# wolearyc/ramannoodle

Measured on AMD Instinct MI355X. Metric: structures/sec (GNN polarizability eval), higher is better.
Workload: dtype f32

## Files before the change

ramannoodle_amd/csrc/api.hip:

```cpp
#include <hip/hip_runtime.h>

#include <algorithm>
#include <chrono>
#include <cmath>
#include <cstdarg>
#include <cstdio>
#include <cstdlib>
#include <cstring>
#include <functional>
#include <memory>
#include <mutex>
#include <string>
#include <thread>
#include <vector>

#include "../../include/rn_potgnn.h"
#include "graph_plan.hpp"
#include "host_runtime.hpp"
#include "increments.hpp"
#include "kernels.hpp"
#include "weight_layout.hpp"

using namespace rn;

// ... 2476 lines not shown
      }
      launch_gather_segments(w, h->step_seg.as<long long>(), (int)(seg.size() / 3), h->step_stage.as<float>(), st);
      HIP_TRY(hipMemcpyAsync(h->step_host, h->step_stage.p, (size_t)total * sizeof(float), hipMemcpyDeviceToHost, st));
      HIP_TRY(hipStreamSynchronize(st));
      for (size_t i = 0; i < seg.size(); i += 3)
        std::memcpy(h->packed.data() + seg[i], h->step_host + seg[i + 1], (size_t)seg[i + 2] * sizeof(float));
    }
    HIP_TRY(hipStreamSynchronize(st));
    h->grads_on_device = false;
    h->train_S = 0;
    h->host_stale = true;
    refresh_pass_flags<float>(h);
    refresh_mfma_mode(h);
    check_ps_fail(h);
  });
}

int rn_potgnn_get_weights(rn_potgnn *h, float *weights, size_t num_weights) {
  if (!h || !weights || num_weights != h->lay.weight_count()) {
    set_error(h, "invalid arguments to get_weights");
    return RN_ERR_INVALID_ARGUMENT;
  }
  return guarded(h, [&]() {
    sync_host(h);
    unpack_weights<float>(h->lay, h->packed.data(), weights, true);
  });
}

int rn_potgnn_set_stat_reducer(rn_potgnn *h, rn_potgnn_reduce_fn fn, void *ctx) {
  if (!h) return RN_ERR_INVALID_ARGUMENT;
  std::lock_guard<std::recursive_mutex> hold(h->lock);
  h->reducer = fn;
  h->reducer_ctx = ctx;
  return RN_OK;
}

double rn_potgnn_train_row_count(const rn_potgnn *h) {
  if (!h) return 0.0;
  std::lock_guard<std::recursive_mutex> hold(h->lock);
  return h->bn_count;
}

int rn_potgnn_train_backward(rn_potgnn *h, const float *dvec6, float *grads) {
  const Checked c = check_pending(h, dvec6 && grads, "train_backward", kHostF32,
                                  "train_backward needs a preceding train_forward (an evaluation or Jacobian call in "
                                  "between discards its tape)");
  if (c.rc != kGo) return c.rc;
  return guarded(h, [&]() { train_backward<float>(h, dvec6, grads); });
}

int rn_potgnn_radius_graph(const double *lattice, const double *positions, int32_t num_atoms,
                           double cutoff, int device, uint8_t *adjacency) {
  if (!lattice || !positions || !adjacency || num_atoms <= 0 || !(cutoff > 0)) {
    set_error<rn_potgnn>(nullptr, "invalid arguments to radius_graph");
    return RN_ERR_INVALID_ARGUMENT;
  }
  int ndev = 0;
  if (hipGetDeviceCount(&ndev) != hipSuccess || device < 0 || device >= ndev) {
    set_error<rn_potgnn>(nullptr, "no usable HIP device (count=%d, requested=%d)", ndev, device);
    return RN_ERR_NO_DEVICE;
  }
  return guarded<rn_potgnn>(nullptr, [&]() {
    HIP_TRY(hipSetDevice(device));
    const size_t n = (size_t)num_atoms;
    DeviceBuf lat, pos, adj;
    lat.ensure(9 * sizeof(double));
    pos.ensure(n * 3 * sizeof(double));
    adj.ensure(n * n);
    HIP_TRY(hipMemcpy(lat.p, lattice, 9 * sizeof(double), hipMemcpyHostToDevice));
    HIP_TRY(hipMemcpy(pos.p, positions, n * 3 * sizeof(double), hipMemcpyHostToDevice));
    launch_radius_graph(lat.as<double>(), pos.as<double>(), num_atoms, (float)cutoff,
                        adj.as<unsigned char>(), nullptr);
    HIP_TRY(hipGetLastError());
    HIP_TRY(hipDeviceSynchronize());
    HIP_TRY(hipMemcpy(adjacency, adj.p, n * n, hipMemcpyDeviceToHost));
  });
}

int rn_potgnn_config_flags(const rn_potgnn *h) {
  if (!h) return -1;
  std::lock_guard<std::recursive_mutex> hold(h->lock);
  int flags = (h->plan.use_fused ? 1 : 0) | ((h->plan.use_fused && h->mfma_f16) ? 4 : 0) | (h->plan.use_narrow ? 8 : 0) |
              ((h->plan.use_fused && h->mfma_range_fallback) ? 16 : 0);
  {
    bool ps = h->plan.use_fused && h->plan.use_ps && !h->f32.pass.empty();
    for (const auto &p : h->f32.pass) ps = ps && (p.c3_fast & 1);
    flags |= ps ? 256 : 0;
  }
  {
    static const bool centred = !(getenv("RN_POTGNN_NODE_CENTRED") && atoi(getenv("RN_POTGNN_NODE_CENTRED")) == 0);
    const bool atom = h->plan.use_fused && h->plan.use_node_fused && h->mfma_f16 && centred && h->g.na_num > 0;
    flags |= atom ? 512 : 0;
    flags |= (atom && (flags & 256) && h->plan.use_readout_fused && h->want_pair_rows && !h->keep_stages) ? 1024 : 0;
    flags |= ((flags & 1024) && h->want_c2_pairs && c2_rows_fit(h)) ? 2048 : 0;
  }
  bool fast = !h->f32.pass.empty();
  for (const auto &p : h->f32.pass) fast = fast && !h->plan.use_narrow && (p.c3_fast & (h->plan.use_fused ? 1 : 2));
  return flags | (fast ? 2 : 0);
}

int rn_potgnn_debug_ps_schedule(const int32_t *rb, const int32_t *re, int32_t num_destinations, int32_t back, int32_t ring_tiles,
                                int32_t *window) {
  if (!rb || !re || num_destinations < 0 || back < 1 || back > 8 || ring_tiles < 1 || ring_tiles > 64) return RN_ERR_INVALID_ARGUMENT;
  int w = 0;
  const bool ok = edge_ps_tile_ok(rb, re, num_destinations, back, ring_tiles, &w);
  if (window) *window = w;
  return ok ? 1 : 0;
}

int64_t rn_potgnn_num_triplets(const rn_potgnn *h) { return h ? h->g.T : -1; }

int rn_potgnn_debug_triplets(rn_potgnn *h, int32_t *idx_i, int32_t *idx_j, int32_t *idx_k,
                             int32_t *slot5, int32_t *slot6) {
  if (!h || !idx_i || !idx_j || !idx_k || !slot5 || !slot6) return RN_ERR_INVALID_ARGUMENT;
  return guarded(h, [&]() {
    const size_t T = (size_t)h->g.T;
    if (T == 0) return;
    DeviceBuf buf;
    buf.ensure(5 * T * sizeof(int));
    int *p = buf.as<int>();
    launch_enum_triplets(h->g, p, p + T, p + 2 * T, p + 3 * T, p + 4 * T, nullptr);
    HIP_TRY(hipGetLastError());
    HIP_TRY(hipDeviceSynchronize());
    int32_t *outs[5] = {idx_i, idx_j, idx_k, slot5, slot6};
    for (int k = 0; k < 5; ++k)
      HIP_TRY(hipMemcpy(outs[k], p + k * T, T * sizeof(int), hipMemcpyDeviceToHost));
  });
}

int rn_potgnn_debug_stage(rn_potgnn *h, int stage, int index, float *out, size_t out_capacity,
                          int64_t *rows, int64_t *cols) {
  if (!h || !out || !rows || !cols) return RN_ERR_INVALID_ARGUMENT;
  std::lock_guard<std::recursive_mutex> hold(h->lock);
  if (h->last_was_f64) {
    set_error(h, "debug_stage only reads the float32 path");
    return RN_ERR_UNSUPPORTED;
  }
  const int S = h->last_chunk_structs;
  Precision<float> &P = h->f32;
  return guarded(h, [&]() {
    HIP_TRY(hipDeviceSynchronize());
    const float *src = nullptr;
    int64_t r = 0, c = 0, ld = 0;
    const int64_t ME = (int64_t)S * h->g.E, MN = (int64_t)S * h->g.N;
    if (stage == 0) {
      src = P.lanes[0].unit4.as<float>(); r = ME; c = 4; ld = 4;
    } else if (stage == 1 || stage == 2) {
      if ((!h->keep_stages && !h->snap_pairs) || index < 0 || index > h->cfg.num_message_passes)
        throw HipError{hipErrorInvalidValue, "stage snapshots need RN_POTGNN_KEEP_STAGES=1 or 2"};
      if (stage == 1) { src = P.snap_node[index].as<float>(); r = MN; c = h->d.Fn; ld = h->d.FnP; }
      else { src = P.snap_edge[index].as<float>(); r = ME; c = h->d.Fe; ld = h->d.FeP; }
    } else if (stage == 3) {
      src = P.lanes[0].bufA.as<float>(); r = ME; c = 12; ld = 32;
    } else {
      throw HipError{hipErrorInvalidValue, "unknown stage"};
    }
    if ((size_t)(r * c) > out_capacity) throw HipError{hipErrorInvalidValue, "out_capacity too small"};
    if (stage == 2 && h->snap_pairs && h->last_pair_rows) {
      std::vector<_Float16> raw((size_t)r * 128);
      HIP_TRY(hipMemcpy(raw.data(), src, raw.size() * sizeof(_Float16), hipMemcpyDeviceToHost));
      for (int64_t i = 0; i < r; ++i)
        for (int64_t k = 0; k < c; ++k) {
          const _Float16 *grp = raw.data() + i * 128 + (k >> 3) * 16;
          out[i * c + k] = (float)grp[k & 7] + (float)grp[8 + (k & 7)];
        }
      *rows = r;
      *cols = c;
      return;
    }
    HIP_TRY(hipMemcpy2D(out, c * sizeof(float), src, ld * sizeof(float), c * sizeof(float), r,
                        hipMemcpyDeviceToHost));
    if (h->last_in_order && r == ME && stage != 1) {
      std::vector<float> tmp(out, out + r * c);
      const int E = h->g.E;
      for (int64_t s = 0; s < S; ++s)
        for (int e = 0; e < E; ++e)
          std::memcpy(out + (s * E + e) * c, tmp.data() + (s * E + h->plan.in_pos[e]) * c, (size_t)c * sizeof(float));
    }
    *rows = r;
    *cols = c;
  });
}

int rn_potgnn_set_profiling(rn_potgnn *h, int enabled) {
  if (!h) return RN_ERR_INVALID_ARGUMENT;
  std::lock_guard<std::recursive_mutex> hold(h->lock);
  resolve_timers(h);
  h->profiling = enabled;
  for (int k = 0; k < K_COUNT; ++k) {
    h->k_ms[k] = 0;
    h->k_launches[k] = 0;
  }
  return RN_OK;
}

int rn_potgnn_kernel_times(rn_potgnn *h, const char **names, double *millis, int64_t *launches,
                           int cap) {
  if (!h || !names || !millis || !launches) return RN_ERR_INVALID_ARGUMENT;
  std::lock_guard<std::recursive_mutex> hold(h->lock);
  (void)hipSetDevice(h->cfg.device);
  resolve_timers(h);
  int n = 0;
  for (int k = 0; k < K_COUNT && n < cap; ++k, ++n) {
    names[n] = kKernelNames[k];
    millis[n] = h->k_ms[k];
    launches[n] = h->k_launches[k];
  }
  return n;
}

}
```

ramannoodle_amd/csrc/kernels_agg.hip:

```cpp
#include <algorithm>
#include <cstdlib>

#include "device_utils.hpp"
#include "kernels.hpp"

namespace rn {

#define RN_DISPATCH_LG(FP, PAD, CALL)                                   \
  do {                                                                  \
    switch ((FP) / 4) {                                                 \
      case 4:  if (PAD) { CALL(4, true); }  else { CALL(4, false); }  break;  \
      case 8:  if (PAD) { CALL(8, true); }  else { CALL(8, false); }  break;  \
      case 16: if (PAD) { CALL(16, true); } else { CALL(16, false); } break;  \
      case 32: if (PAD) { CALL(32, true); } else { CALL(32, false); } break;  \
    }                                                                   \
  } while (0)

template <typename T>
__global__ void setup_kernel(const T *emb, const T *W2, const T *b2, const T *W4,
                             const T *b4, int K, Dims d, T *node_table, const T *b0,
                             const T *bn_w, const T *bn_b, const T *bn_rm, const T *bn_rv,
                             T *scale0, T *shift0) {
  extern __shared__ unsigned char smem_raw[];
  T *h = reinterpret_cast<T *>(smem_raw);
  const int Fn = d.Fn;
  for (int i = threadIdx.x; i < K * Fn; i += blockDim.x) {
    int k = i / Fn, o = i % Fn;
    T acc = b2[o];
    for (int c = 0; c < Fn; ++c) acc += ssp(emb[k * Fn + c]) * W2[o * Fn + c];
    h[i] = ssp(acc);
  }
  __syncthreads();
  for (int i = threadIdx.x; i < K * d.FnP; i += blockDim.x) {
    int k = i / d.FnP, o = i % d.FnP;
    T acc = 0;
    if (o < Fn) {
      acc = b4[o];
      for (int c = 0; c < Fn; ++c) acc += h[k * Fn + c] * W4[o * Fn + c];
    }
    node_table[i] = acc;
  }
  for (int o = threadIdx.x; o < d.FeP; o += blockDim.x) {
    T sc = 0, sh = 0;
    if (o < d.Fe) {
      T inv = (T)1 / sqrt(bn_rv[o] + (T)1e-5);
      sc = inv * bn_w[o];
      sh = (b0[o] - bn_rm[o]) * sc + bn_b[o];
    }
    scale0[o] = sc;
    shift0[o] = sh;
  }
}

template <typename T>
void launch_setup(const T *emb, const T *W2, const T *b2, const T *W4, const T *b4, int K,
                  Dims d, T *node_table, const T *b0, const T *bn_w, const T *bn_b,
                  const T *bn_rm, const T *bn_rv, T *scale0, T *shift0, hipStream_t st) {
  size_t lds = (size_t)K * d.Fn * sizeof(T);
  setup_kernel<T><<<1, 256, lds, st>>>(emb, W2, b2, W4, b4, K, d, node_table, b0, bn_w, bn_b,
                                       bn_rm, bn_rv, scale0, shift0);
}
template void launch_setup<float>(const float *, const float *, const float *, const float *,
                                  const float *, int, Dims, float *, const float *,
                                  const float *, const float *, const float *, const float *,
                                  float *, float *, hipStream_t);
template void launch_setup<double>(const double *, const double *, const double *,
                                   const double *, const double *, int, Dims, double *,
                                   const double *, const double *, const double *,
                                   const double *, const double *, double *, double *,
                                   hipStream_t);

template <typename T, typename PT>
__global__ __launch_bounds__(256) void geom_rbf_kernel(const PT *__restrict__ pos, int S,
                                                       Graph g, const T *__restrict__ lat_base,
                                                       int lat_stride,
                                                       const T *__restrict__ offs, T coef,
                                                       Dims d, T *__restrict__ unit4,
                                                       T *__restrict__ edge0, int in_order) {
  __shared__ T sdist[256];
  const int64_t total = (int64_t)S * g.E;
  const int64_t r0 = (int64_t)blockIdx.x * 256;
  const int64_t row = r0 + threadIdx.x;
  T dist = 0;
  if (row < total) {
    const int s = (int)(row / g.E);
    const int e = in_order ? g.in_edge[(int)(row % g.E)] : (int)(row % g.E);
    const int a = g.edge_a[e], b = g.edge_b[e];
    const T *lat = lat_base + (int64_t)s * lat_stride;
    const PT *pa = pos + ((int64_t)s * g.N + a) * 3;
    const PT *pb = pos + ((int64_t)s * g.N + b) * 3;
    T f[3];
#pragma unroll
    for (int k = 0; k < 3; ++k) f[k] = wrap_min_image((T)pb[k] - (T)pa[k]);
    T c[3];
#pragma unroll
    for (int k = 0; k < 3; ++k) c[k] = f[0] * lat[k] + f[1] * lat[3 + k] + f[2] * lat[6 + k];
    dist = sqrt(c[0] * c[0] + c[1] * c[1] + c[2] * c[2]);
    T *u = unit4 + row * 4;
    u[0] = c[0] / dist;
    u[1] = c[1] / dist;
    u[2] = c[2] / dist;
    u[3] = dist;
  }
  sdist[threadIdx.x] = dist;
  __syncthreads();
  const int c4n = d.FeP / 4;
  for (int i = threadIdx.x; i < 256 * c4n; i += 256) {
    const int r = i / c4n, q = i % c4n;
    if (r0 + r >= total) break;
    const T dd = sdist[r];
    Vec4<T> o;
#pragma unroll
    for (int j = 0; j < 4; ++j) {
      const int col = 4 * q + j;
      T x = dd - offs[col];
      if constexpr (sizeof(T) == 4)
        o.v[j] = (col < d.Fe) ? __builtin_amdgcn_exp2f((coef * 1.4426950408889634f) * (x * x)) : 0.0f;
      else
        o.v[j] = (col < d.Fe) ? exp(coef * (x * x)) : (T)0;
    }
    store4(edge0 + (r0 + r) * d.FeP + 4 * q, o);
  }
}

template <typename T>
void launch_geom_rbf(const double *pos, int S, const Graph &g, const T *lattice, int lat_stride,
                     const T *offsets, T coef, Dims d, T *unit4, T *edge0, hipStream_t st, bool in_order) {
  const int64_t total = (int64_t)S * g.E;
  if (total == 0) return;
  geom_rbf_kernel<T, double><<<(unsigned)((total + 255) / 256), 256, 0, st>>>(pos, S, g, lattice, lat_stride,
                                                                              offsets, coef, d, unit4, edge0, in_order ? 1 : 0);
}
void launch_geom_rbf_pos32(const float *pos, int S, const Graph &g, const float *lattice, int lat_stride,
                           const float *offsets, float coef, Dims d, float *unit4, float *edge0, hipStream_t st, bool in_order) {
  const int64_t total = (int64_t)S * g.E;
  if (total == 0) return;
  geom_rbf_kernel<float, float><<<(unsigned)((total + 255) / 256), 256, 0, st>>>(pos, S, g, lattice, lat_stride,
                                                                                 offsets, coef, d, unit4, edge0, in_order ? 1 : 0);
}
template <typename PT>
__global__ __launch_bounds__(256) void geom_rbf_pairs_kernel(const PT *__restrict__ pos, int S, Graph g,
                                                             const float *__restrict__ lat_base, int lat_stride,
                                                             const float *__restrict__ offs, float coef, Dims d,
                                                             float *__restrict__ unit4, float *__restrict__ edge0) {
  typedef _Float16 h8 __attribute__((ext_vector_type(8)));
  __shared__ float sdist[256];
  const int64_t total = (int64_t)S * g.E;
  const int64_t r0 = (int64_t)blockIdx.x * 256;
  const int64_t row = r0 + threadIdx.x;
  float dist = 0;
  if (row < total) {
    const int s = (int)(row / g.E), e = (int)(row % g.E);
    const int a = g.edge_a[e], b = g.edge_b[e];
    const float *lat = lat_base + (int64_t)s * lat_stride;
    const PT *pa = pos + ((int64_t)s * g.N + a) * 3;
    const PT *pb = pos + ((int64_t)s * g.N + b) * 3;
    float f[3];
#pragma unroll
    for (int k = 0; k < 3; ++k) f[k] = wrap_min_image((float)pb[k] - (float)pa[k]);
    float c[3];
#pragma unroll
    for (int k = 0; k < 3; ++k) c[k] = f[0] * lat[k] + f[1] * lat[3 + k] + f[2] * lat[6 + k];
    dist = sqrt(c[0] * c[0] + c[1] * c[1] + c[2] * c[2]);
    float *u = unit4 + row * 4;
    u[0] = c[0] / dist;
    u[1] = c[1] / dist;
    u[2] = c[2] / dist;
    u[3] = dist;
  }
  sdist[threadIdx.x] = dist;
  __syncthreads();
  for (int i = threadIdx.x; i < 256 * 8; i += 256) {
    const int r = i >> 3, m = i & 7;
    if (r0 + r >= total) break;
    const float dd = sdist[r];
    h8 hi, lo;
#pragma unroll
    for (int j = 0; j < 8; ++j) {
      const int col = 8 * m + j;
      const float x = dd - offs[col];
      const float v = (col < d.Fe) ? __builtin_amdgcn_exp2f((coef * 1.4426950408889634f) * (x * x)) : 0.0f;
      hi[j] = (_Float16)v;
      lo[j] = (_Float16)(v - (float)hi[j]);
    }
    h8 *o = reinterpret_cast<h8 *>(edge0 + (r0 + r) * 64 + 8 * m);
    o[0] = hi;
    o[1] = lo;
  }
}
void launch_geom_rbf_pairs(const double *pos, int S, const Graph &g, const float *lattice, int lat_stride, const float *offsets,
                           float coef, Dims d, float *unit4, float *edge0, hipStream_t st) {
  const int64_t total = (int64_t)S * g.E;
  if (total == 0) return;
  geom_rbf_pairs_kernel<double><<<(unsigned)((total + 255) / 256), 256, 0, st>>>(pos, S, g, lattice, lat_stride, offsets, coef, d,
                                                                                 unit4, edge0);
}
void launch_geom_rbf_pairs_pos32(const float *pos, int S, const Graph &g, const float *lattice, int lat_stride, const float *offsets,
                                 float coef, Dims d, float *unit4, float *edge0, hipStream_t st) {
  const int64_t total = (int64_t)S * g.E;
  if (total == 0) return;
  geom_rbf_pairs_kernel<float><<<(unsigned)((total + 255) / 256), 256, 0, st>>>(pos, S, g, lattice, lat_stride, offsets, coef, d,
                                                                                unit4, edge0);
}
template void launch_geom_rbf<float>(const double *, int, const Graph &, const float *, int,
                                     const float *, float, Dims, float *, float *, hipStream_t, bool);
template void launch_geom_rbf<double>(const double *, int, const Graph &, const double *, int,
                                      const double *, double, Dims, double *, double *,
                                      hipStream_t, bool);

template <typename T>
__global__ void node_init_kernel(const T *__restrict__ table, int S, Graph g, Dims d,
                                 T *__restrict__ node, const int *__restrict__ types) {
  const int c4n = d.FnP / 4;
  const int64_t total = (int64_t)S * g.N * c4n;
  for (int64_t i = (int64_t)blockIdx.x * blockDim.x + threadIdx.x; i < total;
       i += (int64_t)gridDim.x * blockDim.x) {
    const int q = (int)(i % c4n);
    const int64_t rown = i / c4n;
    const int n = (int)(rown % g.N);
    const int ty = types ? types[rown] : g.atom_type[n];
    store4(node + rown * d.FnP + 4 * q, load4<T>(table + ty * d.FnP + 4 * q));
  }
}
template <typename T>
void launch_node_init(const T *table, int S, const Graph &g, Dims d, T *node, const int *types, hipStream_t st) {
  const int64_t total = (int64_t)S * g.N * (d.FnP / 4);
  if (total == 0) return;
  unsigned blocks = (unsigned)((total + 255) / 256);
  if (blocks > 4096) blocks = 4096;
  node_init_kernel<T><<<blocks, 256, 0, st>>>(table, S, g, d, node, types);
}
template void launch_node_init<float>(const float *, int, const Graph &, Dims, float *, const int *, hipStream_t);
template void launch_node_init<double>(const double *, int, const Graph &, Dims, double *, const int *,
                                       hipStream_t);

template <int LG, bool PAD, typename T>
__global__ __launch_bounds__(256) void node_agg_kernel(const T *__restrict__ npc1,
                                                       const T *__restrict__ bc1,
                                                       const T *__restrict__ node_in,
                                                       T *__restrict__ node_out, int S, Graph g,
                                                       Dims d, PassW<T> w) {
  constexpr int FP = LG * 4;
  const int64_t gid = ((int64_t)blockIdx.x * 256 + threadIdx.x) / LG;
  const int q = threadIdx.x % LG;
  if (gid >= (int64_t)S * g.N) return;
  const int s = (int)(gid / g.N), b = (int)(gid % g.N);
  const int nvalid = min(max(d.Fn - 4 * q, 0), 4);
  const T inv2n = (T)1 / (T)(2 * d.Fn), invn = (T)1 / (T)d.Fn;

  LnParams<T> pf{load4<T>(w.c1_norm.g + 4 * q), load4<T>(w.c1_norm.b + 4 * q)};
  LnParams<T> pc{load4<T>(w.c1_norm.g + FP + 4 * q), load4<T>(w.c1_norm.b + FP + 4 * q)};
  const Vec4<T> af = load4<T>(npc1 + gid * (2 * FP) + 4 * q);
  const Vec4<T> ac = load4<T>(npc1 + gid * (2 * FP) + FP + 4 * q);

  Vec4<T> acc{{0, 0, 0, 0}};
  const int beg = g.in_ptr[b], end = g.in_ptr[b + 1];
  const T *base = bc1 + (int64_t)s * g.E * (2 * FP) + 4 * q;
  for (int idx = beg; idx < end; ++idx) {
    const int e = g.in_edge[idx];
    Vec4<T> xf = load4<T>(base + (int64_t)e * (2 * FP));
    Vec4<T> xc = load4<T>(base + (int64_t)e * (2 * FP) + FP);
#pragma unroll
    for (int i = 0; i < 4; ++i) {
      xf.v[i] += af.v[i];
      xc.v[i] += ac.v[i];
    }
    Vec4<T> gt = ln_gate<LG, PAD>(xf, xc, pf, pc, inv2n, nvalid);
#pragma unroll
    for (int i = 0; i < 4; ++i) acc.v[i] += gt.v[i];
  }
  LnParams<T> pn{load4<T>(w.final_norm.g + 4 * q), load4<T>(w.final_norm.b + 4 * q)};
  Vec4<T> ln = ln_row<LG, PAD>(acc, pn, invn, nvalid);
  Vec4<T> old = load4<T>(node_in + gid * FP + 4 * q);
  Vec4<T> out;
#pragma unroll
  for (int i = 0; i < 4; ++i) out.v[i] = acc_tanh(old.v[i] + ln.v[i]);
  store4(node_out + gid * FP + 4 * q, out);
}

template <typename T>
void launch_node_agg(const T *npc1, const T *bc1, const T *node_in, T *node_out, int S,
                     const Graph &g, Dims d, const PassW<T> &w, hipStream_t st) {
  const int lg = d.FnP / 4;
  const int64_t threads = (int64_t)S * g.N * lg;
  if (threads == 0) return;
  const unsigned blocks = (unsigned)((threads + 255) / 256);
  const bool pad = d.Fn != d.FnP;
#define CALL(LGV, PADV) \
  node_agg_kernel<LGV, PADV, T><<<blocks, 256, 0, st>>>(npc1, bc1, node_in, node_out, S, g, d, w)
  RN_DISPATCH_LG(d.FnP, pad, CALL);
#undef CALL
}
template void launch_node_agg<float>(const float *, const float *, const float *, float *, int,
                                     const Graph &, Dims, const PassW<float> &, hipStream_t);
template void launch_node_agg<double>(const double *, const double *, const double *, double *,
                                      int, const Graph &, Dims, const PassW<double> &,
                                      hipStream_t);

template <typename T>
struct GateScale;
template <>
struct GateScale<float> {
  static constexpr float kF = -1.4426950408889634f;
  static constexpr float kC = 2.0f * 1.4426950408889634f;
  static constexpr float kClamp = 43.28f;
};
template <>
struct GateScale<double> {
  static constexpr double kF = -1.4426950408889634;
  static constexpr double kC = 2.0 * 1.4426950408889634;
  static constexpr double kClamp = 115.0;
};
#ifndef RN_EXPERIMENT
#define RN_EXPERIMENT 0
#endif
__device__ __forceinline__ float gate_exp2(float yf, float yc) {
  yc = fminf(fmaxf(yc, -GateScale<float>::kClamp), GateScale<float>::kClamp);
#if RN_EXPERIMENT == 1
  const float e1 = yf * 0.5f + 1.0f, e2 = yc * 0.25f + 1.0f;
  return (e2 - 1.0f) * ((1.0f + e1) * (1.0f + e2));
#else
  const float e1 = fast_exp2(yf), e2 = fast_exp2(yc);
  return (e2 - 1.0f) * fast_rcp((1.0f + e1) * (1.0f + e2));
#endif
}
__device__ __forceinline__ double gate_exp2(double yf, double yc) {
  yc = fmin(fmax(yc, -GateScale<double>::kClamp), GateScale<double>::kClamp);
  const double e1 = exp2(yf), e2 = exp2(yc);
  return (e2 - 1.0) / ((1.0 + e1) * (1.0 + e2));
}

template <int VPL, typename T>
__device__ __forceinline__ void loadv(T (&dst)[VPL], const T *p) {
// ... 513 lines not shown
```

ramannoodle_amd/csrc/kernels_c2_pairs.hip:

```cpp
#include "fused_common.hpp"

namespace rn {

struct C2PairArgs {
  const float *node;
  float *out;
  int64_t M;
  int N, NP;
  const int *pair_a, *pair_b;
  Dims d;
  PassW<float> w;
};

namespace {
constexpr int C2P_THREADS = 256;
}

__global__ __launch_bounds__(C2P_THREADS, 2) void c2_pairs_kernel(C2PairArgs a) {
  __shared__ __attribute__((aligned(16))) float s_bias[2 * FP], s_g1[2 * FP], s_b1[2 * FP], s_g2[FP], s_b2[FP];
  const int tid = threadIdx.x, lane = tid & 63, wave = tid >> 6;
  const int l15 = lane & 15, quad = lane >> 4;
  const float sc2 = a.w.mfma_scale_c[4];
  for (int c = tid; c < 2 * FP; c += C2P_THREADS) {
    s_bias[c] = a.w.c2_bias_c[c] * sc2;
    s_g1[c] = a.w.c2_norm_1.g[c];
    s_b1[c] = a.w.c2_norm_1.b[c];
    if (c < FP) {
      s_g2[c] = a.w.c2_norm_2.g[c];
      s_b2[c] = a.w.c2_norm_2.b[c];
    }
  }
  WaveB<true> bW[4];
#pragma unroll
  for (int p = 0; p < 4; ++p) bW[p].load(a.w.c2_WT_c, 2 * FP, 32 * p, l15, quad, sc2);
  __syncthreads();

  const float inv2n = 1.0f / (float)(2 * a.d.Fe), invn = 1.0f / (float)a.d.Fe;
  const float eps_c2 = 1e-5f * sc2 * sc2;
  const int64_t ntiles = (a.M + 15) / 16, stride = (int64_t)gridDim.x * (C2P_THREADS / 64);

  f32x4 xb[4], xa[4];
  auto fetch = [&](int64_t tile) {
    int64_t row = tile * 16 + l15;
    if (row >= a.M) row = a.M - 1;
    const int64_t s = row / a.NP;
    const int p = (int)(row - s * a.NP);
    const float *nb = a.node + (s * a.N + a.pair_b[p]) * FP + 16 * quad, *na = a.node + (s * a.N + a.pair_a[p]) * FP + 16 * quad;
#pragma unroll
    for (int j = 0; j < 4; ++j) {
      xb[j] = *reinterpret_cast<const f32x4 *>(nb + 4 * j);
      xa[j] = *reinterpret_cast<const f32x4 *>(na + 4 * j);
    }
  };
  int64_t tile = (int64_t)blockIdx.x * (C2P_THREADS / 64) + wave;
  if (tile < ntiles) fetch(tile);
  for (; tile < ntiles; tile += stride) {
    float af[KS];
#pragma unroll
    for (int j = 0; j < 4; ++j) {
      const f32x4 pr = xb[j] * xa[j];
#pragma unroll
      for (int i = 0; i < 4; ++i) af[4 * j + i] = pr[i];
    }
    f16x8 ah[2], al[2];
    split_f16x8(af, ah[0], al[0]);
    split_f16x8(af + 8, ah[1], al[1]);
    if (tile + stride < ntiles) fetch(tile + stride);

    const int lq = launder(lane >> 4);
    f32x4 acc[4][2];
#pragma unroll
    for (int p = 0; p < 4; ++p) {
#pragma unroll
      for (int t = 0; t < 2; ++t) acc[p][t] = *reinterpret_cast<const f32x4 *>(s_bias + 32 * p + 16 * t + 4 * lq);
      bW[p].product_split(ah, al, acc[p]);
    }
    float q = 0.f;
#pragma unroll
    for (int p = 0; p < 4; ++p)
#pragma unroll
      for (int t = 0; t < 2; ++t)
#pragma unroll
        for (int i = 0; i < 4; ++i) q = fmaf(acc[p][t][i], acc[p][t][i], q);
    q = sum_xor32(sum_xor16(q));
    const float rstd2 = fast_rsq(q * inv2n + eps_c2);
    float gv[2][2][4], sum = 0.f;
#pragma unroll
    for (int p = 0; p < 2; ++p)
#pragma unroll
      for (int t = 0; t < 2; ++t) {
        const int c = 32 * p + 16 * t + 4 * lq;
        const Vec4<float> gf = load4<float>(s_g1 + c), bf = load4<float>(s_b1 + c);
        const Vec4<float> gc = load4<float>(s_g1 + FP + c), bc = load4<float>(s_b1 + FP + c);
#pragma unroll
        for (int i = 0; i < 4; ++i) {
          gv[p][t][i] = gate(acc[p][t][i] * rstd2 * gf.v[i] + bf.v[i], acc[p + 2][t][i] * rstd2 * gc.v[i] + bc.v[i]);
          sum += gv[p][t][i];
        }
      }
    const float mean = sum_xor32(sum_xor16(sum)) * invn;
    float qq = 0.f;
#pragma unroll
    for (int p = 0; p < 2; ++p)
#pragma unroll
      for (int t = 0; t < 2; ++t)
#pragma unroll
        for (int i = 0; i < 4; ++i) {
          const int c = 32 * p + 16 * t + 4 * lq + i;
          gv[p][t][i] = c < a.d.Fe ? gv[p][t][i] - mean : 0.f;
          qq = fmaf(gv[p][t][i], gv[p][t][i], qq);
        }
    const float rstd = fast_rsq(sum_xor32(sum_xor16(qq)) * invn + 1e-5f);
    const int64_t row = tile * 16 + l15;
    if (row < a.M) {
#pragma unroll
      for (int p = 0; p < 2; ++p)
#pragma unroll
        for (int t = 0; t < 2; ++t) {
          const int c = 32 * p + 16 * t + 4 * lq;
          const Vec4<float> g2 = load4<float>(s_g2 + c), b2 = load4<float>(s_b2 + c);
          f32x4 y;
#pragma unroll
          for (int i = 0; i < 4; ++i) y[i] = gv[p][t][i] * rstd * g2.v[i] + b2.v[i];
          *reinterpret_cast<f32x4 *>(a.out + row * FP + c) = y;
        }
    }
  }
}

void launch_c2_pairs(const float *node, float *out, int S, const Graph &g, Dims d, const PassW<float> &w, hipStream_t st) {
  const int64_t M = (int64_t)S * g.NP;
  if (M == 0) return;
  C2PairArgs a{node, out, M, g.N, g.NP, g.pair_a, g.pair_b, d, w};
  static int cus = 0;
  if (cus == 0) {
    int dev = 0;
    hipDeviceProp_t prop;
    if (hipGetDevice(&dev) == hipSuccess && hipGetDeviceProperties(&prop, dev) == hipSuccess) cus = prop.multiProcessorCount;
    if (cus <= 0) cus = 256;
  }
  const int64_t ntiles = (M + 15) / 16, per_wg = C2P_THREADS / 64;
  const int64_t grid = std::min<int64_t>((ntiles + per_wg - 1) / per_wg, (int64_t)2 * cus);
  c2_pairs_kernel<<<(unsigned)grid, C2P_THREADS, 0, st>>>(a);
}

}
```

ramannoodle_amd/csrc/kernels_gemm.hip:

```cpp
#include <cstdlib>

#include "device_utils.hpp"
#include "kernels.hpp"

namespace rn {

typedef float f32x16 __attribute__((ext_vector_type(16)));

struct GemmArgs {
  const float *X;
  int ldx;
  int accum;
  int64_t M;
  const float *WT;
  int NOUT;
  float *Y;
  const float *scale, *shift;
  const float *node;
  const int *edge_a, *edge_b;
  int N, E;
};

template <int KP, int WN, int TN, int AMODE, int EPI, bool EXT = false>
__global__ __launch_bounds__(256) void rowgemm_mfma_kernel(GemmArgs a) {
// ... 157 lines not shown
  if (first < num_tiles) fetch(first);
  for (int it = 0; it < tiles_per_wave; ++it) {
    const int64_t tile = first + it;
    if (tile >= num_tiles) break;
    float afrag[32];
#pragma unroll
    for (int j = 0; j < 8; ++j) {
      float4 v = nxt[j];
      if (AMODE == 1) v = make_float4(v.x * nxt2[j].x, v.y * nxt2[j].y, v.z * nxt2[j].z, v.w * nxt2[j].w);
      afrag[4 * j] = v.x; afrag[4 * j + 1] = v.y; afrag[4 * j + 2] = v.z; afrag[4 * j + 3] = v.w;
    }
    if (it + 1 < tiles_per_wave && tile + 1 < num_tiles) fetch(tile + 1);
    const int64_t row0 = tile * 32;
#pragma unroll 1
    for (int nt = 0; nt < NS / 32; ++nt) {
      const float *wp = wt + (nt * 32 + l31) * LDW + 32 * h;
      f32x16 acc;
#pragma unroll
      for (int r = 0; r < 16; ++r) acc[r] = 0.f;
#pragma unroll
      for (int j = 0; j < 8; ++j) {
        const float4 b = *reinterpret_cast<const float4 *>(wp + 4 * j);
        acc = __builtin_amdgcn_mfma_f32_32x32x2f32(afrag[4 * j], b.x, acc, 0, 0, 0);
        acc = __builtin_amdgcn_mfma_f32_32x32x2f32(afrag[4 * j + 1], b.y, acc, 0, 0, 0);
        acc = __builtin_amdgcn_mfma_f32_32x32x2f32(afrag[4 * j + 2], b.z, acc, 0, 0, 0);
        acc = __builtin_amdgcn_mfma_f32_32x32x2f32(afrag[4 * j + 3], b.w, acc, 0, 0, 0);
      }
      const int col = ncol0 + nt * 32 + l31;
      const float sc = (EPI == 2) ? a.scale[col] : 1.0f;
      const float sh = (EPI >= 1) ? a.shift[col] : 0.0f;
#pragma unroll
      for (int r = 0; r < 16; ++r) {
        const int64_t row = row0 + (r & 3) + 8 * (r >> 2) + 4 * h;
        if (row < a.M) {
          float v = acc[r];
          if (EPI == 1) v += sh;
          if (EPI == 2) v = ssp_fast(v * sc + sh);
          a.Y[row * a.NOUT + col] = v;
        }
      }
    }
  }
}

static bool launch_stream64(const GemmArgs &a, int amode, int epi, hipStream_t st) {
  static const int enabled = getenv("RN_POTGNN_GEMM_STREAM") ? atoi(getenv("RN_POTGNN_GEMM_STREAM")) : 0;
  if (!enabled || a.NOUT % 128 != 0 || a.M < 4096) return false;
  const int64_t tiles = (a.M + 31) / 32;
  static const int tpw_env = getenv("RN_POTGNN_GEMM_TPW") ? atoi(getenv("RN_POTGNN_GEMM_TPW")) : 4;
  const int tpw = tpw_env < 1 ? 1 : tpw_env;
  const dim3 grid((unsigned)((tiles + 4 * tpw - 1) / (4 * tpw)), (unsigned)(a.NOUT / 128));
#define RN_ST(AM, EP) rowgemm_stream64_kernel<AM, EP><<<grid, 256, 0, st>>>(a, tpw)
  if (amode == 0) {
    if (epi == 0) RN_ST(0, 0);
    else if (epi == 1) RN_ST(0, 1);
    else RN_ST(0, 2);
  } else {
    if (epi == 0) RN_ST(1, 0);
    else RN_ST(1, 1);
  }
#undef RN_ST
  return true;
}

template <int KP, int WN, int TN>
static void launch_mfma_cfg(const GemmArgs &a, int amode, int epi, dim3 grid, hipStream_t st) {
#define RN_GEMM(AM, EP) rowgemm_mfma_kernel<KP, WN, TN, AM, EP><<<grid, 256, 0, st>>>(a)
  if (amode == 0) {
    if (epi == 0) RN_GEMM(0, 0);
    else if (epi == 1) RN_GEMM(0, 1);
    else RN_GEMM(0, 2);
  } else {
    if (epi == 0) RN_GEMM(1, 0);
    else RN_GEMM(1, 1);
  }
#undef RN_GEMM
}

template <int KP>
static void launch_mfma_ext(const GemmArgs &a, hipStream_t st) {
  int slice = 32;
  if (a.NOUT % 64 == 0) slice = 64;
  if (a.NOUT % 128 == 0) slice = 128;
  const int64_t tiles = (a.M + 127) / 128;
  dim3 grid((unsigned)(tiles < 2048 ? tiles : 2048), (unsigned)(a.NOUT / slice));
  switch (slice) {
    case 32: rowgemm_mfma_kernel<KP, 1, 1, 0, 0, true><<<grid, 256, 0, st>>>(a); break;
    case 64: rowgemm_mfma_kernel<KP, 2, 1, 0, 0, true><<<grid, 256, 0, st>>>(a); break;
    case 128: rowgemm_mfma_kernel<KP, 4, 1, 0, 0, true><<<grid, 256, 0, st>>>(a); break;
  }
}

template <int KP>
static void launch_mfma_kp(const GemmArgs &a, int amode, int epi, hipStream_t st) {
  int slice = 32;
  if (a.NOUT % 64 == 0) slice = 64;
  if (a.NOUT % 128 == 0) slice = 128;
  static const int max_slice = getenv("RN_POTGNN_GEMM_MAXSLICE") ? atoi(getenv("RN_POTGNN_GEMM_MAXSLICE")) : 256;
  if (a.NOUT % 256 == 0 && KP <= 64 && max_slice >= 256) slice = 256;
  const int64_t tiles = (a.M + 127) / 128;
  dim3 grid((unsigned)(tiles < 2048 ? tiles : 2048), (unsigned)(a.NOUT / slice));
  switch (slice) {
    case 32: launch_mfma_cfg<KP, 1, 1>(a, amode, epi, grid, st); break;
    case 64: launch_mfma_cfg<KP, 2, 1>(a, amode, epi, grid, st); break;
    case 128: launch_mfma_cfg<KP, 4, 1>(a, amode, epi, grid, st); break;
    case 256:
      if constexpr (KP <= 64) launch_mfma_cfg<KP, 4, 2>(a, amode, epi, grid, st);
      break;
  }
}

template <>
void launch_rowgemm<float>(const float *X, int64_t M, int KP, const float *WT, int NOUT, float *Y,
                           const float *scale, const float *shift, bool act, int amode,
                           const float *node, const Graph &g, hipStream_t st) {
  if (M == 0) return;
  GemmArgs a{X, KP, 0, M, WT, NOUT, Y, scale, shift, node, g.edge_a, g.edge_b, g.N, g.E};
  const int epi = act ? 2 : (shift ? 1 : 0);
  switch (KP) {
    case 16: launch_mfma_kp<16>(a, amode, epi, st); break;
    case 32: launch_mfma_kp<32>(a, amode, epi, st); break;
    case 64:
      if (!launch_stream64(a, amode, epi, st)) launch_mfma_kp<64>(a, amode, epi, st);
      break;
    case 128: launch_mfma_kp<128>(a, amode, epi, st); break;
  }
}

bool launch_rowgemm_blocks(const float *X, int ldx, int N, int64_t M, const float *Wt, int NOUT,
                           float *Y, bool accumulate, const Graph &g, hipStream_t st) {
  if (M == 0) return true;
  if (NOUT % 32 != 0 || N % 16 != 0) return false;
  int bk = 128;
  while (N % bk != 0) bk /= 2;
  for (int off = 0; off < N; off += bk) {
    GemmArgs a{X + off, ldx, (accumulate || off > 0) ? 1 : 0, M, Wt + (size_t)off * NOUT, NOUT, Y,
               nullptr, nullptr, nullptr, g.edge_a, g.edge_b, g.N, g.E};
    switch (bk) {
      case 16: launch_mfma_ext<16>(a, st); break;
      case 32: launch_mfma_ext<32>(a, st); break;
      case 64: launch_mfma_ext<64>(a, st); break;
      case 128: launch_mfma_ext<128>(a, st); break;
    }
  }
  return true;
}

typedef _Float16 gf16x8 __attribute__((ext_vector_type(8)));
typedef _Float16 gf16x4 __attribute__((ext_vector_type(4)));
template <int KB, int NTW, int AMODE>
__global__ __launch_bounds__(256, 2) void rowgemm_split_kernel(GemmArgs a) {
  __shared__ __attribute__((aligned(16))) gf16x8 atile[2][KB][2][2][64];
  __shared__ float s_inv[2][16];
  const int tid = threadIdx.x, lane = tid & 63, wave = tid >> 6;
  const int l15 = lane & 15, quad = lane >> 4;
  const int col0 = blockIdx.y * (64 * NTW) + wave * (16 * NTW);

  gf16x8 wh[KB][NTW][2], wl[KB][NTW][2];
  float winv[KB];
#pragma unroll
  for (int kb = 0; kb < KB; ++kb) {
    float tmp[NTW][2][8];
    float m = 0.f;
#pragma unroll
    for (int t = 0; t < NTW; ++t)
#pragma unroll
      for (int s2 = 0; s2 < 2; ++s2)
#pragma unroll
        for (int j = 0; j < 8; ++j) {
          tmp[t][s2][j] = a.WT[(int64_t)(64 * kb + 16 * quad + 8 * s2 + j) * a.NOUT + col0 + 16 * t + l15];
          m = fmaxf(m, fabsf(tmp[t][s2][j]));
        }
#pragma unroll
    for (int sft = 1; sft < 64; sft <<= 1) m = fmaxf(m, __shfl_xor(m, sft));
    const float sw = mfma_prescale(m);
    winv[kb] = 1.0f / sw;
#pragma unroll
    for (int t = 0; t < NTW; ++t)
#pragma unroll
      for (int s2 = 0; s2 < 2; ++s2) {
#pragma unroll
        for (int j = 0; j < 8; ++j) tmp[t][s2][j] *= sw;
        split_f16x8(tmp[t][s2], wh[kb][t][s2], wl[kb][t][s2]);
      }
  }

  constexpr int LPR = 16 * KB;
  const int64_t ntiles = (a.M + 15) / 16;
  float4 nxt[KB];
  auto fetch = [&](int64_t tile) {
#pragma unroll
    for (int j = 0; j < KB; ++j) {
      const int idx = j * 64 + lane;
      int64_t row = tile * 16 + 4 * wave + idx / LPR;
      if (row >= a.M) row = a.M - 1;
      const int p = idx % LPR;
      if (AMODE == 0) {
        nxt[j] = *reinterpret_cast<const float4 *>(a.X + row * a.ldx + 4 * p);
      } else {
        const int64_t s = row / a.E;
        const int e = (int)(row - s * a.E);
        const float4 x = *reinterpret_cast<const float4 *>(a.node + (s * a.N + a.edge_b[e]) * (64 * KB) + 4 * p);
        const float4 y = *reinterpret_cast<const float4 *>(a.node + (s * a.N + a.edge_a[e]) * (64 * KB) + 4 * p);
        nxt[j] = make_float4(x.x * y.x, x.y * y.y, x.z * y.z, x.w * y.w);
      }
    }
  };
  auto stage = [&](int b) {
#pragma unroll
    for (int j = 0; j < KB; ++j) {
      const int idx = j * 64 + lane;
      const int rowl = 4 * wave + idx / LPR, p = idx % LPR;
      float4 v = nxt[j];
      float m = fmaxf(fmaxf(fabsf(v.x), fabsf(v.y)), fmaxf(fabsf(v.z), fabsf(v.w)));
#pragma unroll
      for (int sft = 1; sft < LPR; sft <<= 1) m = fmaxf(m, __shfl_xor(m, sft));
      const float sr = mfma_prescale(m);
      if (p == 0) s_inv[b][rowl] = 1.0f / sr;
      const float x[4] = {v.x * sr, v.y * sr, v.z * sr, v.w * sr};
      gf16x4 hi, lo;
#pragma unroll
      for (int k = 0; k < 4; ++k) {
        hi[k] = (_Float16)x[k];
        lo[k] = (_Float16)(x[k] - (float)hi[k]);
      }
      const int kb = p >> 4, qd = (p >> 2) & 3, s2 = (p >> 1) & 1, half = p & 1;
      gf16x4 *dh = reinterpret_cast<gf16x4 *>(&atile[b][kb][s2][0][rowl * 4 + qd]) + half;
      gf16x4 *dl = reinterpret_cast<gf16x4 *>(&atile[b][kb][s2][1][rowl * 4 + qd]) + half;
      *dh = hi;
      *dl = lo;
    }
  };
  if ((int64_t)blockIdx.x < ntiles) fetch(blockIdx.x);
  int b = 0;
  for (int64_t tile = blockIdx.x; tile < ntiles; tile += gridDim.x, b ^= 1) {
    stage(b);
    if (tile + gridDim.x < ntiles) fetch(tile + gridDim.x);
    const int64_t row = tile * 16 + l15;
    const bool live = row < a.M;
    float4 old[NTW];
    if (a.accum && live) {
#pragma unroll
      for (int t = 0; t < NTW; ++t) old[t] = *reinterpret_cast<const float4 *>(a.Y + row * a.NOUT + col0 + 16 * t + 4 * quad);
    }
    __syncthreads();
    const float inv_sr = s_inv[b][l15];
    f32x4_t tot[NTW];
#pragma unroll
    for (int t = 0; t < NTW; ++t) tot[t] = f32x4_t{0.f, 0.f, 0.f, 0.f};
#pragma unroll
    for (int kb = 0; kb < KB; ++kb) {
      const gf16x8 ah0 = atile[b][kb][0][0][l15 * 4 + quad], al0 = atile[b][kb][0][1][l15 * 4 + quad];
      const gf16x8 ah1 = atile[b][kb][1][0][l15 * 4 + quad], al1 = atile[b][kb][1][1][l15 * 4 + quad];
      const float scale = winv[kb] * inv_sr;
#pragma unroll
      for (int t = 0; t < NTW; ++t) {
        f32x4_t acc = {0.f, 0.f, 0.f, 0.f};
        acc = mfma_split3(wh[kb][t][0], wl[kb][t][0], ah0, al0, acc);
        acc = mfma_split3(wh[kb][t][1], wl[kb][t][1], ah1, al1, acc);
        tot[t] += acc * scale;
      }
    }
    if (live) {
#pragma unroll
      for (int t = 0; t < NTW; ++t) {
        const int col = col0 + 16 * t + 4 * quad;
        float4 v = make_float4(tot[t][0], tot[t][1], tot[t][2], tot[t][3]);
        if (a.shift) {
          const float4 bb = *reinterpret_cast<const float4 *>(a.shift + col);
          v.x += bb.x; v.y += bb.y; v.z += bb.z; v.w += bb.w;
        }
        if (a.accum) {
          v.x += old[t].x; v.y += old[t].y; v.z += old[t].z; v.w += old[t].w;
        }
        *reinterpret_cast<float4 *>(a.Y + row * a.NOUT + col) = v;
      }
    }
  }
}

bool launch_rowgemm_split(const float *X, int ldx, int K, int64_t M, const float *Wt, int NOUT, float *Y,
                          bool accumulate, const float *bias, int amode, const float *node, const Graph &g,
                          hipStream_t st) {
  if (M == 0) return true;
  static const bool off = getenv("RN_POTGNN_BWD_SPLIT_GEMM") && atoi(getenv("RN_POTGNN_BWD_SPLIT_GEMM")) == 0;
  if (off || K % 64 != 0 || K > 256 || K == 192 || NOUT % 64 != 0 || (amode == 1 && K > 128)) return false;
  GemmArgs a{X, ldx, accumulate ? 1 : 0, M, Wt, NOUT, Y, nullptr, bias, node, g.edge_a, g.edge_b, g.N, g.E};
  const int kb = K / 64;
  int ntw = 1;
  if (kb == 1 && NOUT % 256 == 0) ntw = 4;
  else if (kb <= 2 && NOUT % 128 == 0) ntw = 2;
  const int64_t ntiles = (M + 15) / 16;
  static int cus = 0;
  if (cus == 0) {
    int dev = 0;
    hipDeviceProp_t prop;
    if (hipGetDevice(&dev) == hipSuccess && hipGetDeviceProperties(&prop, dev) == hipSuccess) cus = prop.multiProcessorCount;
    if (cus <= 0) cus = 256;
  }
  static const int wgs_per_cu = getenv("RN_POTGNN_SPLIT_GEMM_WGS") ? std::max(1, atoi(getenv("RN_POTGNN_SPLIT_GEMM_WGS"))) : 4;
  const dim3 grid((unsigned)std::min<int64_t>(ntiles, (int64_t)wgs_per_cu * cus), (unsigned)(NOUT / (64 * ntw)));
#define RN_SPLIT(KBV, NTWV)                                                             \
  do {                                                                                  \
    if (amode == 1) rowgemm_split_kernel<1, NTWV, 1><<<grid, 256, 0, st>>>(a);          \
    else rowgemm_split_kernel<KBV, NTWV, 0><<<grid, 256, 0, st>>>(a);                   \
  } while (0)
  if (kb == 1 && ntw == 4) RN_SPLIT(1, 4);
  else if (kb == 1 && ntw == 2) RN_SPLIT(1, 2);
  else if (kb == 1) RN_SPLIT(1, 1);
  else if (kb == 2 && ntw == 2) {
    if (amode == 1) rowgemm_split_kernel<2, 2, 1><<<grid, 256, 0, st>>>(a);
    else rowgemm_split_kernel<2, 2, 0><<<grid, 256, 0, st>>>(a);
  } else if (kb == 2) {
    if (amode == 1) rowgemm_split_kernel<2, 1, 1><<<grid, 256, 0, st>>>(a);
    else rowgemm_split_kernel<2, 1, 0><<<grid, 256, 0, st>>>(a);
  }
  else { if (amode == 1) return false; rowgemm_split_kernel<4, 1, 0><<<grid, 256, 0, st>>>(a); }
#undef RN_SPLIT
  return true;
}

__global__ __launch_bounds__(256) void rowgemm_f64_kernel(const double *X, int64_t M, int KP,
                                                          const double *WT, int NOUT, double *Y,
                                                          const double *scale, const double *shift,
                                                          int epi, int amode, const double *node,
                                                          Graph g) {
  extern __shared__ __attribute__((aligned(16))) unsigned char smem_raw[];
  double *xs = reinterpret_cast<double *>(smem_raw);
  const int64_t num_tiles = (M + 31) / 32;
  for (int64_t tile = blockIdx.x; tile < num_tiles; tile += gridDim.x) {
    const int64_t row0 = tile * 32;
    for (int i = threadIdx.x; i < 32 * KP; i += 256) {
      const int r = i / KP, c = i % KP;
      const int64_t row = row0 + r;
      double v = 0;
      if (row < M) {
        if (amode == 0) {
          v = X[row * KP + c];
        } else {
          const int64_t s = row / g.E;
          const int e = (int)(row % g.E);
          v = node[(s * g.N + g.edge_b[e]) * KP + c] * node[(s * g.N + g.edge_a[e]) * KP + c];
        }
      }
      xs[i] = v;
    }
    __syncthreads();
    for (int col = threadIdx.x; col < NOUT; col += 256) {
      double acc[32];
#pragma unroll
      for (int r = 0; r < 32; ++r) acc[r] = 0;
      for (int k = 0; k < KP; ++k) {
        const double wv = WT[(int64_t)k * NOUT + col];
#pragma unroll
        for (int r = 0; r < 32; ++r) acc[r] += xs[r * KP + k] * wv;
      }
      const double sc = (epi == 2) ? scale[col] : 1.0;
      const double sh = (epi >= 1) ? shift[col] : 0.0;
#pragma unroll
      for (int r = 0; r < 32; ++r) {
        const int64_t row = row0 + r;
        if (row < M) {
          double v = acc[r];
          if (epi == 1) v += sh;
          if (epi == 2) v = ssp(v * sc + sh);
          Y[row * NOUT + col] = v;
        }
      }
    }
    __syncthreads();
  }
}

typedef double f64x4_t __attribute__((ext_vector_type(4)));
template <int KQ, int NTW>
__global__ __launch_bounds__(256) void rowgemm_f64_mfma_kernel(const double *__restrict__ X, int64_t M,
                                                               const double *__restrict__ WT, int NOUT,
                                                               double *__restrict__ Y, const double *__restrict__ scale,
                                                               const double *__restrict__ shift, int epi, int amode,
                                                               const double *__restrict__ node, Graph g) {
  constexpr int K = 4 * KQ;
  const int lane = threadIdx.x & 63, wave = threadIdx.x >> 6;
  const int l15 = lane & 15, quad = lane >> 4;
  const int col0 = blockIdx.y * (64 * NTW) + wave * (16 * NTW);
  if (col0 >= NOUT) return;
  double w[NTW][KQ];
#pragma unroll
  for (int t = 0; t < NTW; ++t)
#pragma unroll
    for (int ks = 0; ks < KQ; ++ks) w[t][ks] = WT[(int64_t)(KQ * quad + ks) * NOUT + col0 + 16 * t + l15];
  const int64_t ntiles = (M + 15) / 16;
  double nxt[KQ];
  auto fetch = [&](int64_t tile) {
    int64_t row = tile * 16 + l15;
    if (row >= M) row = M - 1;
    if (amode == 0) {
      const double *p = X + row * K + KQ * quad;
#pragma unroll
      for (int ks = 0; ks < KQ; ks += 2) {
        const double2 v = *reinterpret_cast<const double2 *>(p + ks);
        nxt[ks] = v.x;
        nxt[ks + 1] = v.y;
      }
    } else {
      const int64_t s = row / g.E;
      const int e = (int)(row - s * g.E);
      const double *pb = node + (s * g.N + g.edge_b[e]) * K + KQ * quad, *pa = node + (s * g.N + g.edge_a[e]) * K + KQ * quad;
#pragma unroll
      for (int ks = 0; ks < KQ; ks += 2) {
        const double2 x = *reinterpret_cast<const double2 *>(pb + ks), y = *reinterpret_cast<const double2 *>(pa + ks);
        nxt[ks] = x.x * y.x;
        nxt[ks + 1] = x.y * y.y;
      }
    }
  };
  if ((int64_t)blockIdx.x < ntiles) fetch(blockIdx.x);
  for (int64_t tile = blockIdx.x; tile < ntiles; tile += gridDim.x) {
    double x[KQ];
#pragma unroll
    for (int ks = 0; ks < KQ; ++ks) x[ks] = nxt[ks];
    if (tile + gridDim.x < ntiles) fetch(tile + gridDim.x);
    f64x4_t acc[NTW];
#pragma unroll
// ... 77 lines not shown
```

Measured before the change: 64000.

## Stage GEMM output rows through LDS, hoist bias and RBF offsets, add stage-4 snapshot

In the split row-GEMM, for the KB=1/NTW=2 case the output tile is staged in shared memory so each wave writes full contiguous rows with float4 stores. The bias vectors are loaded once per block instead of once per tile. The geometry/RBF kernel hoists the per-lane Gaussian offsets and the lattice/position loads into registers, and the pairs LayerNorm kernel clamps out-of-range rows instead of branching on them. A new stage-4 debug snapshot path is also added. The staged store adds a shared buffer and an extra barrier per tile, and the clamped rows can cause redundant writes to the last row.

```diff
diff --git a/ramannoodle_amd/csrc/api.hip b/ramannoodle_amd/csrc/api.hip
--- a/ramannoodle_amd/csrc/api.hip
+++ b/ramannoodle_amd/csrc/api.hip
@@ -2652,6 +2652,10 @@
       else { src = P.snap_edge[index].as<float>(); r = ME; c = h->d.Fe; ld = h->d.FeP; }
     } else if (stage == 3) {
       src = P.lanes[0].bufA.as<float>(); r = ME; c = 12; ld = 32;
+    } else if (stage == 4) {
+      if ((!h->keep_stages && !h->snap_pairs) || index < 0 || index > h->cfg.num_message_passes)
+        throw HipError{hipErrorInvalidValue, "stage snapshots need RN_POTGNN_KEEP_STAGES=1 or 2"};
+      src = P.snap_edge[index].as<float>(); r = ME; c = h->d.FeP; ld = h->d.FeP;
     } else {
       throw HipError{hipErrorInvalidValue, "unknown stage"};
     }
@@ -2670,7 +2674,7 @@
     }
     HIP_TRY(hipMemcpy2D(out, c * sizeof(float), src, ld * sizeof(float), c * sizeof(float), r,
                         hipMemcpyDeviceToHost));
-    if (h->last_in_order && r == ME && stage != 1) {
+    if (h->last_in_order && r == ME && stage != 1 && stage != 4) {
       std::vector<float> tmp(out, out + r * c);
       const int E = h->g.E;
       for (int64_t s = 0; s < S; ++s)
diff --git a/ramannoodle_amd/csrc/kernels_agg.hip b/ramannoodle_amd/csrc/kernels_agg.hip
--- a/ramannoodle_amd/csrc/kernels_agg.hip
+++ b/ramannoodle_amd/csrc/kernels_agg.hip
@@ -148,6 +148,10 @@
   const int64_t total = (int64_t)S * g.E;
   const int64_t r0 = (int64_t)blockIdx.x * 256;
   const int64_t row = r0 + threadIdx.x;
+  const int lane = threadIdx.x & 63, m = lane & 7;
+  float mu[8];
+#pragma unroll
+  for (int j = 0; j < 8; ++j) mu[j] = offs[8 * m + j];
   float dist = 0;
   if (row < total) {
     const int s = (int)(row / g.E), e = (int)(row % g.E);
@@ -155,12 +159,17 @@
     const float *lat = lat_base + (int64_t)s * lat_stride;
     const PT *pa = pos + ((int64_t)s * g.N + a) * 3;
     const PT *pb = pos + ((int64_t)s * g.N + b) * 3;
+    float xa[3], xb[3], lt[9];
+#pragma unroll
+    for (int k = 0; k < 3; ++k) xa[k] = (float)pa[k], xb[k] = (float)pb[k];
+#pragma unroll
+    for (int k = 0; k < 9; ++k) lt[k] = lat[k];
     float f[3];
 #pragma unroll
-    for (int k = 0; k < 3; ++k) f[k] = wrap_min_image((float)pb[k] - (float)pa[k]);
+    for (int k = 0; k < 3; ++k) f[k] = wrap_min_image(xb[k] - xa[k]);
     float c[3];
 #pragma unroll
-    for (int k = 0; k < 3; ++k) c[k] = f[0] * lat[k] + f[1] * lat[3 + k] + f[2] * lat[6 + k];
+    for (int k = 0; k < 3; ++k) c[k] = f[0] * lt[k] + f[1] * lt[3 + k] + f[2] * lt[6 + k];
     dist = sqrt(c[0] * c[0] + c[1] * c[1] + c[2] * c[2]);
     float *u = unit4 + row * 4;
     u[0] = c[0] / dist;
@@ -171,14 +180,14 @@
   sdist[threadIdx.x] = dist;
   __syncthreads();
   for (int i = threadIdx.x; i < 256 * 8; i += 256) {
-    const int r = i >> 3, m = i & 7;
+    const int r = i >> 3;
     if (r0 + r >= total) break;
     const float dd = sdist[r];
     h8 hi, lo;
 #pragma unroll
     for (int j = 0; j < 8; ++j) {
       const int col = 8 * m + j;
-      const float x = dd - offs[col];
+      const float x = dd - mu[j];
       const float v = (col < d.Fe) ? __builtin_amdgcn_exp2f((coef * 1.4426950408889634f) * (x * x)) : 0.0f;
       hi[j] = (_Float16)v;
       lo[j] = (_Float16)(v - (float)hi[j]);
diff --git a/ramannoodle_amd/csrc/kernels_c2_pairs.hip b/ramannoodle_amd/csrc/kernels_c2_pairs.hip
--- a/ramannoodle_amd/csrc/kernels_c2_pairs.hip
+++ b/ramannoodle_amd/csrc/kernels_c2_pairs.hip
@@ -111,8 +111,8 @@
           qq = fmaf(gv[p][t][i], gv[p][t][i], qq);
         }
     const float rstd = fast_rsq(sum_xor32(sum_xor16(qq)) * invn + 1e-5f);
-    const int64_t row = tile * 16 + l15;
-    if (row < a.M) {
+    const int64_t row = tile * 16 + l15 < a.M ? tile * 16 + l15 : a.M - 1;
+    {
 #pragma unroll
       for (int p = 0; p < 2; ++p)
 #pragma unroll
diff --git a/ramannoodle_amd/csrc/kernels_gemm.hip b/ramannoodle_amd/csrc/kernels_gemm.hip
--- a/ramannoodle_amd/csrc/kernels_gemm.hip
+++ b/ramannoodle_amd/csrc/kernels_gemm.hip
@@ -333,6 +333,8 @@
 __global__ __launch_bounds__(256, 2) void rowgemm_split_kernel(GemmArgs a) {
   __shared__ __attribute__((aligned(16))) gf16x8 atile[2][KB][2][2][64];
   __shared__ float s_inv[2][16];
+  constexpr bool ROWOUT = KB == 1 && NTW == 2 && AMODE == 0;
+  __shared__ __attribute__((aligned(16))) float otile[ROWOUT ? 16 : 1][132];
   const int tid = threadIdx.x, lane = tid & 63, wave = tid >> 6;
   const int l15 = lane & 15, quad = lane >> 4;
   const int col0 = blockIdx.y * (64 * NTW) + wave * (16 * NTW);
@@ -412,6 +414,10 @@
       *dl = lo;
     }
   };
+  float4 bias[NTW];
+#pragma unroll
+  for (int t = 0; t < NTW; ++t)
+    bias[t] = a.shift ? *reinterpret_cast<const float4 *>(a.shift + col0 + 16 * t + 4 * quad) : make_float4(0.f, 0.f, 0.f, 0.f);
   if ((int64_t)blockIdx.x < ntiles) fetch(blockIdx.x);
   int b = 0;
   for (int64_t tile = blockIdx.x; tile < ntiles; tile += gridDim.x, b ^= 1) {
@@ -442,14 +448,35 @@
         tot[t] += acc * scale;
       }
     }
-    if (live) {
+    bool stored = false;
+    if constexpr (ROWOUT) if (!a.accum) {
+      stored = true;
+#pragma unroll
+      for (int t = 0; t < NTW; ++t) {
+        const int c = wave * (16 * NTW) + 16 * t + 4 * quad;
+        float4 v = make_float4(tot[t][0], tot[t][1], tot[t][2], tot[t][3]);
+        if (a.shift) {
+          v.x += bias[t].x; v.y += bias[t].y; v.z += bias[t].z; v.w += bias[t].w;
+        }
+        *reinterpret_cast<float4 *>(&otile[l15][c]) = v;
+      }
+      __syncthreads();
+#pragma unroll
+      for (int i = 0; i < 2; ++i) {
+        const int rowl = 4 * wave + 2 * i + (lane >> 5), c = 4 * (lane & 31);
+        const int64_t orow = tile * 16 + rowl;
+        if (orow < a.M)
+          *reinterpret_cast<float4 *>(a.Y + orow * a.NOUT + blockIdx.y * (64 * NTW) + c) =
+              *reinterpret_cast<const float4 *>(&otile[rowl][c]);
+      }
+    }
+    if (live && !stored) {
 #pragma unroll
       for (int t = 0; t < NTW; ++t) {
         const int col = col0 + 16 * t + 4 * quad;
         float4 v = make_float4(tot[t][0], tot[t][1], tot[t][2], tot[t][3]);
         if (a.shift) {
-          const float4 bb = *reinterpret_cast<const float4 *>(a.shift + col);
-          v.x += bb.x; v.y += bb.y; v.z += bb.z; v.w += bb.w;
+          v.x += bias[t].x; v.y += bias[t].y; v.z += bias[t].z; v.w += bias[t].w;
         }
         if (a.accum) {
           v.x += old[t].x; v.y += old[t].y; v.z += old[t].z; v.w += old[t].w;
```

Result: faster. 65110, median of 6 (+1.7%).
